# ortk95/planetmapper

Measured on NVIDIA B200. Metric: full-backplane Mpix/s (FP64) + mapped-cube voxels/s at 1-8 B200 vs host CPU, higher is better.
Workload: dtype f64

## Files before the change

### planetmapper_b200/csrc/backplane_kernels.cu

```cuda
#include "pm_device.cuh"
#include "pm_kernels.h"

#include <cstdlib>

namespace pm {

constexpr int kPerThread = 4;
#ifndef PM_IMG_PARAM_CTAS
#define PM_IMG_PARAM_CTAS 4
#endif
constexpr int kImgParamCtas = PM_IMG_PARAM_CTAS;

__device__ __forceinline__ int slot(uint64_t mask, int k) { return __popcll(mask & (bit(k) - 1ull)); }

struct PlaneOffsets {
    int64_t byte_off[PM_N_PLANES];
    int64_t frame_stride;
};
static PlaneOffsets make_plane_offsets(uint64_t mask, int64_t plane_stride) {
    PlaneOffsets po;
    int slot = 0;
    for (int k = 0; k < PM_N_PLANES; k++) {
        po.byte_off[k] = (int64_t)slot * plane_stride * (int64_t)sizeof(double);
        if (mask & bit(k)) slot++;
// ... 44 lines not shown
    const uint32_t j = (k + 1u) >> 1;
    if (j <= min(lo, hi)) return (k & 1u) ? centre + j : centre - j;
    return lo < hi ? k : n_tiles - 1u - k;
}
template <bool kSky, uint64_t kFixedMask>
__global__ void __launch_bounds__(kBlock, kImgParamCtas) backplanes_img_param_kernel(
    const __grid_constant__ FrameD fs, uint32_t nx, uint32_t npx, int per_thread, uint32_t centre_tile, uint64_t mask,
    const __grid_constant__ PlaneOffsets po, double *__restrict__ out) {
    img_tile<kSky, kFixedMask>(fs, centre_out_tile(blockIdx.x, gridDim.x, centre_tile), nx, npx, per_thread, mask,
                               po, out);
}

template <bool kSky, bool kRingAll>
__global__ void __launch_bounds__(kBlock, 4) backplanes_points_param_kernel(const __grid_constant__ FrameD fs,
                                                                            const double *__restrict__ x_in,
                                                                            const double *__restrict__ y_in,
                                                                            int64_t n, uint64_t mask,
                                                                            const __grid_constant__ PlaneOffsets po,
                                                                            double *__restrict__ out) {
    const int64_t first = (int64_t)blockIdx.x * (kBlock * kPerThread) + threadIdx.x;
#pragma unroll 1
    for (int r = 0; r < kPerThread; r++) {
        const int64_t idx = first + r * kBlock;
        if (idx >= n) break;
        PlaneSink sink{reinterpret_cast<char *>(out + idx), po};
        image_point<kSky, kRingAll>(fs, __ldg(x_in + idx), __ldg(y_in + idx), mask, sink);
    }
}

constexpr uint64_t kXYMapMask = bit(PM_PIXEL_X) | bit(PM_PIXEL_Y);

template <uint64_t kFixedMask>
__device__ __forceinline__ void map_tile(const FrameD &fs, const double *__restrict__ lon_in,
                                         const double *__restrict__ lat_in, int64_t n, uint64_t mask,
                                         const PlaneOffsets &po, double *__restrict__ out) {
    const int64_t first = (int64_t)blockIdx.x * (kBlock * kPerThread) + threadIdx.x;
#pragma unroll 1
    for (int r = 0; r < kPerThread; r++) {
        const int64_t idx = first + r * kBlock;
        if (idx >= n) break;
        PlaneSink sink{reinterpret_cast<char *>(out + idx), po};
        map_cell<kFixedMask>(fs, __ldg(lon_in + idx), __ldg(lat_in + idx), mask, sink);
    }
}

template <uint64_t kFixedMask>
__global__ void __launch_bounds__(kBlock, 4) backplanes_map_kernel(const PMFrame *__restrict__ frame,
                                                                   const double *__restrict__ lon_in,
                                                                   const double *__restrict__ lat_in,
                                                                   int64_t n, uint64_t mask,
                                                                   const __grid_constant__ PlaneOffsets po,
                                                                   double *__restrict__ out) {
    __shared__ FrameD fs;
    load_frame(fs, frame + blockIdx.y);
    map_tile<kFixedMask>(fs, lon_in, lat_in, n, mask, po, out + (int64_t)blockIdx.y * po.frame_stride);
}

template <uint64_t kFixedMask>
__global__ void __launch_bounds__(kBlock, 4) backplanes_map_param_kernel(const __grid_constant__ FrameD fs,
                                                                         const double *__restrict__ lon_in,
                                                                         const double *__restrict__ lat_in,
                                                                         int64_t n, uint64_t mask,
                                                                         const __grid_constant__ PlaneOffsets po,
                                                                         double *__restrict__ out) {
    map_tile<kFixedMask>(fs, lon_in, lat_in, n, mask, po, out);
}

__global__ void __launch_bounds__(kBlock, 4) xy2lonlat_kernel(const PMFrame *__restrict__ frame,
                                                              const double *__restrict__ xs,
                                                              const double *__restrict__ ys, int64_t n,
                                                              double *__restrict__ lon_out,
                                                              double *__restrict__ lat_out,
                                                              unsigned long long *__restrict__ n_missed) {
    __shared__ FrameD fs;
    load_frame(fs, frame);
    unsigned long long missed = 0;
    const int64_t first = (int64_t)blockIdx.x * (kBlock * kPerThread) + threadIdx.x;
#pragma unroll 1
    for (int r = 0; r < kPerThread; r++) {
        const int64_t idx = first + r * kBlock;
        if (idx >= n) break;
        const double x = xs[idx], y = ys[idx];
        double lon = NAN, lat = NAN;
        if (fabs(x) < INFINITY && fabs(y) < INFINITY) {
            if (!xy2lonlat_point(fs, x, y, lon, lat)) missed++;
        }
        lon_out[idx] = lon;
        lat_out[idx] = lat;
    }
    if (n_missed) {
        for (int o = 16; o > 0; o >>= 1) missed += __shfl_down_sync(0xffffffffu, missed, o);
        if ((threadIdx.x & 31) == 0 && missed) atomicAdd(n_missed, missed);
    }
}

__global__ void __launch_bounds__(kBlock, 4) lonlat2xy_kernel(const PMFrame *__restrict__ frame,
                                                              const double *__restrict__ lons,
                                                              const double *__restrict__ lats, int64_t n,
                                                              double alt, uint32_t flags,
                                                              double *__restrict__ x_out,
                                                              double *__restrict__ y_out) {
    __shared__ FrameD fs;
    load_frame(fs, frame);
    const int64_t first = (int64_t)blockIdx.x * (kBlock * kPerThread) + threadIdx.x;
#pragma unroll 1
    for (int r = 0; r < kPerThread; r++) {
        const int64_t idx = first + r * kBlock;
        if (idx >= n) break;
        const double lon = lons[idx], lat = lats[idx];
        double x = NAN, y = NAN;
        if (fabs(lon) < INFINITY && fabs(lat) < INFINITY)
            lonlat2xy_point(fs, lon, lat, alt, (flags & PM_FLAG_NOT_VISIBLE_NAN) != 0,
                            (flags & PM_FLAG_PLANETOCENTRIC) != 0, x, y);
        x_out[idx] = x;
        y_out[idx] = y;
    }
}

__global__ void __launch_bounds__(kBlock, 4) transform_kernel(const PMFrame *__restrict__ frame,
                                                              const __grid_constant__ TransformAux aux, int use_aux,
                                                              int src, int dst, const double *__restrict__ a_in,
                                                              const double *__restrict__ b_in, int64_t n, double alt,
                                                              uint32_t flags, double *__restrict__ a_out,
                                                              double *__restrict__ b_out,
                                                              unsigned long long *__restrict__ n_missed) {
    __shared__ FrameD fs;
    __shared__ TransformAux ax;
    load_frame(fs, frame);
    if (threadIdx.x < 13) {
        double v;
        if (use_aux) {
            v = threadIdx.x < 9 ? aux.Mc[threadIdx.x] : aux.km2ang[threadIdx.x - 9];
        } else if (threadIdx.x < 9) {
            v = fs.f.M[threadIdx.x];
        } else {
            const double *m = fs.f.ang2km;
            const double det = fma(m[0], m[3], -m[1] * m[2]);
            const int k = threadIdx.x - 9;
            v = (k == 0 ? m[3] : k == 1 ? -m[1] : k == 2 ? -m[2] : m[0]) / det;
        }
        (threadIdx.x < 9 ? ax.Mc[threadIdx.x] : ax.km2ang[threadIdx.x - 9]) = v;
    }
    __syncthreads();
    unsigned long long missed = 0;
    const int64_t first = (int64_t)blockIdx.x * (kBlock * kPerThread) + threadIdx.x;
#pragma unroll 1
    for (int r = 0; r < kPerThread; r++) {
        const int64_t idx = first + r * kBlock;
        if (idx >= n) break;
        double oa, ob;
        if (!point_transform(fs, ax, src, dst, a_in[idx], b_in[idx], alt, flags, oa, ob)) missed++;
        a_out[idx] = oa;
        b_out[idx] = ob;
    }
    if (n_missed) {
        for (int o = 16; o > 0; o >>= 1) missed += __shfl_down_sync(0xffffffffu, missed, o);
        if ((threadIdx.x & 31) == 0 && missed) atomicAdd(n_missed, missed);
    }
}

template <int kKind>
__global__ void __launch_bounds__(256) fp64_probe_kernel(double *out, const double *in, int iters, double m, double c) {
    double a[8], b[8], d[8];
#pragma unroll
    for (int i = 0; i < 8; i++) {
        a[i] = threadIdx.x * 1e-9 + i;
        b[i] = kKind ? in[(threadIdx.x + 2 * i + 1) & 63] : m;
        d[i] = kKind ? in[(threadIdx.x + 3 * i + 2) & 63] * 1e-12 : c;
    }
#pragma unroll 1
    for (int it = 0; it < iters; it++) {
#pragma unroll
        for (int i = 0; i < 8; i++) a[i] = kKind ? fma(a[i], b[i], d[i]) : fma(a[i], m, c);
    }
    double s = a[0] + a[1] + a[2] + a[3] + a[4] + a[5] + a[6] + a[7];
    if (s == 123.456) out[0] = s;
}

__global__ void math_probe_kernel(int kind, const double *__restrict__ a, const double *__restrict__ b,
                                  int64_t n, double *__restrict__ out) {
    const int64_t i = (int64_t)blockIdx.x * blockDim.x + threadIdx.x;
// ... 174 lines not shown
```

### planetmapper_b200/csrc/pm_device.cuh

```cuda
#pragma once

#include "../../include/pm_b200.h"
#include "pm_math.cuh"

namespace pm {

struct V3 {
    double x, y, z;
};

PM_HD V3 mk(double x, double y, double z) { return V3{x, y, z}; }
PM_HD V3 operator+(V3 a, V3 b) { return mk(a.x + b.x, a.y + b.y, a.z + b.z); }
PM_HD V3 operator-(V3 a, V3 b) { return mk(a.x - b.x, a.y - b.y, a.z - b.z); }
PM_HD V3 operator-(V3 a) { return mk(-a.x, -a.y, -a.z); }
PM_HD V3 operator*(double s, V3 a) { return mk(s * a.x, s * a.y, s * a.z); }
PM_HD double dot(V3 a, V3 b) { return fma(a.x, b.x, fma(a.y, b.y, a.z * b.z)); }
PM_HD V3 cross(V3 a, V3 b) {
    return mk(fma(a.y, b.z, -a.z * b.y), fma(a.z, b.x, -a.x * b.z), fma(a.x, b.y, -a.y * b.x));
}
PM_HD V3 mul3(V3 a, const double *s) { return mk(a.x * s[0], a.y * s[1], a.z * s[2]); }
PM_HD V3 axpy(double s, V3 b, V3 a) { return mk(fma(s, b.x, a.x), fma(s, b.y, a.y), fma(s, b.z, a.z)); }
PM_HD double norm(V3 a) { return fast_sqrt_lite(dot(a, a)); }
PM_HD V3 ld3(const double *p) { return mk(p[0], p[1], p[2]); }
PM_HD bool finite3(V3 a) { return fabs(a.x) < INFINITY && fabs(a.y) < INFINITY && fabs(a.z) < INFINITY; }
PM_HD V3 mxv(const double *m, V3 v) {
    return mk(fma(m[0], v.x, fma(m[1], v.y, m[2] * v.z)), fma(m[3], v.x, fma(m[4], v.y, m[5] * v.z)),
              fma(m[6], v.x, fma(m[7], v.y, m[8] * v.z)));
}
PM_HD V3 mtxv(const double *m, V3 v) {
    return mk(fma(m[0], v.x, fma(m[3], v.y, m[6] * v.z)), fma(m[1], v.x, fma(m[4], v.y, m[7] * v.z)),
              fma(m[2], v.x, fma(m[5], v.y, m[8] * v.z)));
}
PM_HD_NOINLINE double pymod360_slow(double a) {
    double r = ::fmod(a, 360.0);
    if (r != 0.0 && r < 0.0) r += 360.0;
    return r;
}
PM_HD double pymod360(double a) { return (a >= 0.0 && a < 360.0) ? a : pymod360_slow(a); }

struct FrameD {
    PMFrame f;
    double inv_c;
    double inv_r[3];
    double nw[3];
    double k[3];
    double wn;
    double rp;
    double e2, ep2;
    double inv_omf2;
    double omf;
    double P0b[3], VTb[3], ATb[3], VOb[3], S0b[3], VSb[3];
    double G[9];
    double y0[3];
    double y0m2;
    double As[6];
    double inv_kmpa;
    int biaxial;
    int pad_;
};

constexpr int kDeriveItems = 13;

PM_HD double ex_mul(double a, double b) {
#ifdef __CUDA_ARCH__
    return __dmul_rn(a, b);
#else
    return a * b;
#endif
}
PM_HD double ex_add(double a, double b) {
#ifdef __CUDA_ARCH__
    return __dadd_rn(a, b);
#else
    return a + b;
#endif
}
PM_HD double ex_div(double a, double b) {
#ifdef __CUDA_ARCH__
    return __ddiv_rn(a, b);
#else
    return a / b;
#endif
}
PM_HD double ex_sqrt(double a) {
#ifdef __CUDA_ARCH__
    return __dsqrt_rn(a);
#else
    return ::sqrt(a);
#endif
}
PM_HD double ex_dot3(double a0, double b0, double a1, double b1, double a2, double b2) {
    return ex_add(ex_add(ex_mul(a0, b0), ex_mul(a1, b1)), ex_mul(a2, b2));
}

PM_HD void derive_frame_item(FrameD &s, int item) {
    const PMFrame &f = s.f;
    if (item >= 3 && item <= 8) {
        const double *src = item == 3 ? f.P0 : item == 4 ? f.VT : item == 5 ? f.AT : item == 6 ? f.VO : item == 7 ? f.S0 : f.VS;
        double *dst = item == 3 ? s.P0b : item == 4 ? s.VTb : item == 5 ? s.ATb : item == 6 ? s.VOb : item == 7 ? s.S0b : s.VSb;
        for (int r = 0; r < 3; r++)
            dst[r] = ex_dot3(f.R0[3 * r], src[0], f.R0[3 * r + 1], src[1], f.R0[3 * r + 2], src[2]);
        if (item == 3) {
            for (int r = 0; r < 3; r++) s.y0[r] = ex_mul(-dst[r], ex_div(1.0, f.radii[r]));
            s.y0m2 = fma(s.y0[0], s.y0[0], fma(s.y0[1], s.y0[1], ex_mul(s.y0[2], s.y0[2])));
        }
    } else if (item >= 9 && item <= 11) {
        const int r = item - 9;
        for (int c = 0; c < 3; c++)
            s.G[3 * r + c] = ex_dot3(f.R0[3 * r], f.M[3 * c], f.R0[3 * r + 1], f.M[3 * c + 1], f.R0[3 * r + 2], f.M[3 * c + 2]);
    } else if (item == 12) {
        const double sc = kRpd / 3600.0;
        for (int c = 0; c < 3; c++) {
            s.As[c] = -ex_mul(f.A[c], sc);
            s.As[3 + c] = ex_mul(f.A[3 + c], sc);
        }
        s.inv_kmpa = ex_div(1.0, f.km_per_arcsec);
    } else if (item == 0) {
        s.inv_c = ex_div(1.0, f.clight);
        const double w2 = ex_dot3(f.omega[0], f.omega[0], f.omega[1], f.omega[1], f.omega[2], f.omega[2]);
        const double wn = ex_sqrt(w2);
        s.wn = wn;
        s.k[0] = wn > 0.0 ? ex_div(f.omega[0], wn) : 0.0;
        s.k[1] = wn > 0.0 ? ex_div(f.omega[1], wn) : 0.0;
        s.k[2] = wn > 0.0 ? ex_div(f.omega[2], wn) : 0.0;
    } else if (item == 1) {
        const double a = f.radii[0], b = f.radii[1], c = f.radii[2];
        s.inv_r[0] = ex_div(1.0, a);
        s.inv_r[1] = ex_div(1.0, b);
        s.inv_r[2] = ex_div(1.0, c);
        const double m = fmin(a, fmin(b, c));
        const double ma = ex_div(m, a), mb = ex_div(m, b), mc = ex_div(m, c);
        s.nw[0] = ex_mul(ma, ma);
        s.nw[1] = ex_mul(mb, mb);
        s.nw[2] = ex_mul(mc, mc);
    } else if (item == 2) {
        const double rp = ex_add(f.re, -ex_mul(f.f, f.re));
        const double re2 = ex_mul(f.re, f.re), rp2 = ex_mul(rp, rp);
        const double omf = ex_add(1.0, -f.f);
        s.rp = rp;
        s.e2 = ex_add(1.0, -ex_div(rp2, re2));
        s.ep2 = ex_add(ex_div(re2, rp2), -1.0);
        s.omf = omf;
        s.inv_omf2 = ex_div(1.0, ex_mul(omf, omf));
        s.biaxial = (f.radii[0] == f.radii[1]) && (f.re == f.radii[0]) && (fabs(rp - f.radii[2]) <= 4e-16 * f.radii[2]);
        s.pad_ = 0;
    }
}

#ifdef __CUDACC__
__device__ __forceinline__ void load_frame(FrameD &s, const PMFrame *__restrict__ g) {
    const double *src = reinterpret_cast<const double *>(g);
    double *dst = reinterpret_cast<double *>(&s.f);
    for (int i = threadIdx.x; i < PM_FRAME_NDOUBLES; i += blockDim.x) dst[i] = __ldg(src + i);
    __syncthreads();
    const int w = threadIdx.x >> 5, l = threadIdx.x & 31;
    int item = -1;
    if (blockDim.x >= 128) {
        if (w == 0 && l < 6) item = 3 + l;
        else if (w == 1 && l < 4) item = 9 + l;
        else if (w == 2 && l < 2) item = l;
        else if (w == 3 && l == 0) item = 2;
    } else if (threadIdx.x < kDeriveItems) {
        item = threadIdx.x;
    }
    if (item >= 0) derive_frame_item(s, item);
    __syncthreads();
}
#endif
inline void load_frame_host(FrameD &s, const PMFrame *g) {
    s.f = *g;
    for (int i = 0; i < kDeriveItems; i++) derive_frame_item(s, i);
}

#ifndef PM_GRAZING_COS2
#define PM_GRAZING_COS2 3.0e-3
#endif
constexpr double kGrazingCos2 = PM_GRAZING_COS2;

enum PixC {
    kPixDt1Min = 0,
    kPixGrazing = 1,
    kPixInv60 = 2,
    kPixInv3600 = 3,
    kPixRpd = 4,
    kPixBetaMax = 5,
};
PM_DEV_TABLE(kPixC, 6, 1.0e-6, kGrazingCos2, 1.0 / 60.0, 1.0 / 3600.0, kRpd, 1.0e-3)

struct Rot {
    double s, omc;
};
PM_HD Rot make_rot(const FrameD &fs, double dt) {
    const double th = fs.wn * dt;
    Rot r;
    if (fabs(th) < 0.001953125) {
        const double z = th * th;
        r.s = th * fma(z, fma(z, PM_T(kTinyC)[0], PM_T(kTinyC)[2]), 1.0);
        r.omc = z * fma(z, fma(z, -PM_T(kTinyC)[1], -PM_T(kTinyC)[3]), 0.5);
    } else {
        double sh, ch;
        sincos_lib(0.5 * th, &sh, &ch);
        r.s = 2.0 * sh * ch;
        r.omc = 2.0 * sh * sh;
    }
    return r;
}
PM_HD V3 spin_fwd(const FrameD &fs, Rot r, V3 w) {
    const V3 k = ld3(fs.k);
    const V3 c = cross(w, k);
    const double kw = dot(k, w);
    const V3 t = mk(fma(k.x, kw, -w.x), fma(k.y, kw, -w.y), fma(k.z, kw, -w.z));
    return axpy(r.omc, t, axpy(r.s, c, w));
}
PM_HD V3 spin_bwd_c(const FrameD &fs, Rot r, V3 u, V3 kxu) {
    const V3 k = ld3(fs.k);
    const double ku = dot(k, u);
    const V3 t = mk(fma(k.x, ku, -u.x), fma(k.y, ku, -u.y), fma(k.z, ku, -u.z));
    return axpy(r.omc, t, axpy(r.s, kxu, u));
}
PM_HD V3 spin_bwd(const FrameD &fs, Rot r, V3 u) { return spin_bwd_c(fs, r, u, cross(ld3(fs.k), u)); }
PM_HD V3 to_body(const FrameD &fs, Rot r, V3 v) { return spin_fwd(fs, r, mxv(fs.f.R0, v)); }
PM_HD V3 from_body(const FrameD &fs, Rot r, V3 u) { return mtxv(fs.f.R0, spin_bwd(fs, r, u)); }
PM_HD V3 target_pos_b(const FrameD &fs, double dt) {
    const double h = 0.5 * dt * dt;
    return mk(fma(fs.ATb[0], h, fma(fs.VTb[0], dt, fs.P0b[0])), fma(fs.ATb[1], h, fma(fs.VTb[1], dt, fs.P0b[1])),
              fma(fs.ATb[2], h, fma(fs.VTb[2], dt, fs.P0b[2])));
}

PM_HD void recrad_angles(V3 v, double &ra, double &dec) {
    dec = fast_atan2_xpos(v.z, fast_sqrt(fma(v.x, v.x, v.y * v.y)));
    double lon = fast_atan2(v.y, v.x);
    if (lon < 0.0) lon += kTwoPi;
    ra = lon;
}
PM_HD V3 radrec1(double ra, double dec) {
    double sr, cr, sd, cd;
    sincos_full(ra, sr, cr);
    sincos_full(dec, sd, cd);
    return mk(cr * cd, sr * cd, sd);
}
PM_HD double vsep(V3 a, V3 b) { return fast_atan2_ypos(norm(cross(a, b)), dot(a, b)); }

struct RayHit {
    V3 pp;
    double ixx;
    double a;
    double t;
    double cos2;
};
PM_HD bool surfpt_y(const FrameD &fs, V3 y, double ym2, V3 u, V3 &p, RayHit &hit) {
    const V3 x = mul3(u, fs.inv_r);
    const double xx = dot(x, x), yx = dot(y, x);
    if (!(xx > 0.0)) return false;
    const double ixx = fast_rcp(xx);
    const double a = -(yx * ixx);
    const V3 pp = axpy(a, x, y);
    const double pm2 = dot(pp, pp);
    if (!(pm2 < INFINITY)) return false;
    hit.pp = pp;
    hit.ixx = ixx;
    hit.a = a;
    hit.cos2 = 1.0 - pm2;
    double h;
    if (ym2 > 1.0) {
        if (pm2 > 1.0) return false;
        if (yx > 0.0) return false;
        h = -fast_sqrt_lite((1.0 - pm2) * ixx);
    } else if (ym2 == 1.0) {
        h = -a;
    } else {
        h = fast_sqrt_lite(fmax(0.0, 1.0 - pm2) * ixx);
    }
    hit.t = a + h;
    p = mul3(axpy(h, x, pp), fs.f.radii);
    return true;
}
PM_HD bool surfpt(const FrameD &fs, V3 o, V3 u, V3 &p, RayHit &hit) {
    const V3 y = mul3(o, fs.inv_r);
    return surfpt_y(fs, y, dot(y, y), u, p, hit);
}

struct Intercept {
    V3 p;
    V3 u;
    Rot r;
    double dt;
    double L;
    double lt;
};

PM_HD_NOINLINE bool sincpt_converge(const FrameD &fs, V3 u0, double &dt, V3 &p, double &range) {
    const PMFrame &f = fs.f;
    for (int it = 0; it < 8; it++) {
        const Rot r = make_rot(fs, dt);
        const V3 o = spin_fwd(fs, r, -target_pos_b(fs, dt));
        RayHit hit;
        if (!surfpt(fs, o, spin_fwd(fs, r, u0), p, hit)) return false;
        range = hit.t;
        const double t = dt + f.t_ref;
        const double t_new = f.et - hit.t * fs.inv_c;
        if (!(fabs(t_new - t) > 1.0e-17 * fabs(t_new))) break;
        dt = t_new - f.t_ref;
    }
    return true;
}

PM_HD bool sincpt(const FrameD &fs, V3 u0, Intercept &it) {
    const PMFrame &f = fs.f;
    V3 p1, p2;
    RayHit h1, h2;
    if (!surfpt_y(fs, ld3(fs.y0), fs.y0m2, u0, p1, h1)) return false;
    const double lt1 = h1.t * fs.inv_c;

    const double dt1 = (f.et - lt1) - f.t_ref;
    const Rot r1 = make_rot(fs, dt1);
    if (!surfpt(fs, spin_fwd(fs, r1, -target_pos_b(fs, dt1)), spin_fwd(fs, r1, u0), p2, h2)) return false;
    const double lt2 = h2.t * fs.inv_c;

    double dt = (f.et - lt2) - f.t_ref;
    V3 p;
    double L;
    if (fabs(dt1) > PM_T(kPixC)[kPixDt1Min] && h2.cos2 > PM_T(kPixC)[kPixGrazing]) {
        const double lam = fast_div_lite(dt - dt1, dt1 - (dt - dt1));
        dt = fma(lam, dt1, dt1) + f.t_ref;
        dt -= f.t_ref;
        const V3 pps = axpy(lam, h2.pp - h1.pp, h2.pp);
        const double hs = fast_sqrt_lite(fmax(1.0 - dot(pps, pps), 0.0) * fma(lam, h2.ixx - h1.ixx, h2.ixx));
        L = fma(lam, h2.a - h1.a, h2.a) - hs;
        it.r = make_rot(fs, dt);
        it.u = spin_fwd(fs, it.r, u0);
        p = axpy(-hs, it.u, mul3(pps, fs.f.radii));
    } else {
        double dt_c = dt, L_c;
        V3 p_c;
        if (!sincpt_converge(fs, u0, dt_c, p_c, L_c)) return false;
        dt = dt_c;
        p = p_c;
        L = L_c;
        it.r = make_rot(fs, dt);
        it.u = spin_fwd(fs, it.r, u0);
    }
    it.p = p;
    it.dt = dt;
    it.L = L;
    it.lt = L * fs.inv_c;
    return true;
}

PM_HD void geodetic_general(const FrameD &fs, double rho, double z, double &lat, double &alt) {
    const PMFrame &f = fs.f;
    if (f.f == 0.0) {
        lat = fast_atan2_xpos(z, rho);
        alt = fast_sqrt(fma(rho, rho, z * z)) - f.re;
        return;
    }
    double sb = f.re * z, cb = fs.rp * rho;
    double n = fast_rsqrt(fma(sb, sb, cb * cb) + sqrt_guard());
    sb *= n;
    cb *= n;
    double num = z, den = rho;
#pragma unroll 1
    for (int i = 0; i < 8; i++) {
        num = fma(fs.ep2 * fs.rp, sb * sb * sb, z);
        den = fma(-fs.e2 * f.re, cb * cb * cb, rho);
        double nsb = fs.omf * num, ncb = den;
        n = fast_rsqrt(fma(nsb, nsb, ncb * ncb) + sqrt_guard());
        nsb *= n;
        ncb *= n;
        const double change = fabs(nsb - sb) + fabs(ncb - cb);
// ... 63 lines not shown
PM_HD double local_solar_time(const PMFrame &f, double lon_deg) {
    double ang = f.lon_sign * (lon_deg * PM_T(kPixC)[kPixRpd]) - f.sun_lon_lst;
    if (f.prograde == 0.0) ang = -ang;
    const double k = floor(ang * PM_T(kMisc)[8]);
    ang = fma(-k, PM_T(kMisc)[7], ang);
    if (ang < 0.0) ang += PM_T(kMisc)[7];
    if (ang >= PM_T(kMisc)[7]) ang -= PM_T(kMisc)[7];
    double sec = fma(ang, 86400.0 / kTwoPi, 43200.0);
    if (sec >= 86400.0) sec -= 86400.0;
    const int isec = (int)sec;
    const int hr = isec / 3600, rem = isec - hr * 3600;
    const int mn = rem / 60, sc = rem - mn * 60;
    const double dm = (double)mn, ds = (double)sc;
    double qm = dm * PM_T(kPixC)[kPixInv60];
    qm = fma(fma(-60.0, qm, dm), PM_T(kPixC)[kPixInv60], qm);
    double qs = ds * PM_T(kPixC)[kPixInv3600];
    qs = fma(fma(-3600.0, qs, ds), PM_T(kPixC)[kPixInv3600], qs);
    return ((double)hr + qm) + qs;
}

PM_HD_NOINLINE double doppler_factor_closed(double beta) { return fast_sqrt(fast_div(1.0 + beta, 1.0 - beta)); }
PM_HD_NOINLINE double light_time_rate_closed(double a, double b, double c) { return fast_div(a - b, c + a); }
PM_HD double doppler_factor(const FrameD &fs, double rv) {
    const double beta = rv * fs.inv_c;
    if (fabs(beta) < PM_T(kPixC)[kPixBetaMax])
        return fma(beta, fma(beta, fma(beta, fma(beta, fma(beta, 0.375, 0.375), 0.5), 0.5), 1.0), 1.0);
    return doppler_factor_closed(beta);
}

PM_HD double radial_velocity(const FrameD &fs, double a, double b) {
    const double ac = a * fs.inv_c;
    double dlt = (a - b) * fs.inv_c * fma(ac, ac - 1.0, 1.0);
    if (!(fabs(ac) < PM_T(kPixC)[kPixBetaMax])) dlt = light_time_rate_closed(a, b, fs.f.clight);
    return fma(-dlt, a, a) - b;
}

struct Illum {
    double phase, incdnc, emissn, azimuth;
};
PM_HD void illum_angles(V3 n, V3 s, V3 e, bool want_az, Illum &out) {
    const V3 cse = cross(s, e), cns = cross(n, s), cne = cross(n, e);
    const double dse = dot(s, e), dns = dot(n, s), dne = dot(n, e);
    const double mns = norm(cns), mne = norm(cne);
    out.phase = fast_atan2_ypos(norm(cse), dse);
    out.incdnc = fast_atan2_ypos(mns, dns);
    out.emissn = fast_atan2_ypos(mne, dne);
    if (want_az) {
        const double nn = dot(n, n);
        const double a = fma(dse, nn, -dne * dns);
        out.azimuth = fast_atan2_ypos(fast_sqrt_pos(nn) * fabs(dot(n, cse)), -a);
    }
}

PM_HD void illum_at(const FrameD &fs, V3 p, V3 p0 , V3 e, Rot r, double dt, bool want_az,
                    Illum &out) {
    const PMFrame &f = fs.f;
    const double h = 0.5 * dt * dt;
    const V3 base = mk(fs.S0b[0] - fma(fs.ATb[0], h, fma(fs.VTb[0], dt, p0.x)),
                       fs.S0b[1] - fma(fs.ATb[1], h, fma(fs.VTb[1], dt, p0.y)),
                       fs.S0b[2] - fma(fs.ATb[2], h, fma(fs.VTb[2], dt, p0.z)));
    const V3 VSb = ld3(fs.VSb);
    V3 sv = axpy(dt, VSb, base);
    const double lts = fast_sqrt_pos(dot(sv, sv)) * fs.inv_c;
    sv = axpy(dt - (lts - f.lts0), VSb, base);
    const V3 s_b = spin_fwd(fs, r, sv);
    const V3 n = mul3(p, fs.nw);
    illum_angles(n, s_b, e, want_az, out);
}

struct PointGeom {
    V3 p0;
    V3 X0;
    Rot r;
    double dt, L, lt;
};
PM_HD void point_geom(const FrameD &fs, V3 p, PointGeom &g) {
    const PMFrame &f = fs.f;
    double lt = norm(ld3(fs.P0b) + p) * fs.inv_c;
#pragma unroll 1
    for (int pass = 0; pass < 2; pass++) {
        const double dt = (f.et - lt) - f.t_ref;
        const Rot r = make_rot(fs, dt);
        const V3 p0 = spin_bwd(fs, r, p);
        const V3 X0 = target_pos_b(fs, dt) + p0;
        const double L = norm(X0);
        lt = L * fs.inv_c;
        g.p0 = p0;
        g.X0 = X0;
        g.r = r;
        g.dt = dt;
        g.L = L;
        g.lt = lt;
    }
}
PM_HD double point_rv(const FrameD &fs, V3 p, const PointGeom &g) {
    const double iL = fast_rcp(g.L);
    const V3 ph0 = iL * g.X0;
    const V3 vt = axpy(g.dt, ld3(fs.ATb), ld3(fs.VTb));
    const V3 vrot0 = spin_bwd(fs, g.r, cross(ld3(fs.f.omega), p));
    const double a = dot(vt + vrot0, ph0);
    const double b = dot(ld3(fs.VOb), ph0);
    return radial_velocity(fs, a, b);
}

PM_HD V3 xy2ray_local(const FrameD &fs, double x, double y) {
    const double ra = fma(fs.As[0], x, fma(fs.As[1], y, fs.As[2]));
    const double dec = fma(fs.As[3], x, fma(fs.As[4], y, fs.As[5]));
    double sr, cr, sd, cd;
    sincos_small2(ra, dec, sr, cr, sd, cd);
    return mk(cr * cd, sr * cd, sd);
}

PM_HD void obsvec2angular(const PMFrame &f, V3 ov, double &ax, double &ay) {
    double ra, dec;
    recrad_angles(mxv(f.M, ov), ra, dec);
    double x = pymod360(-(ra * kDpr));
    if (x > 180.0) x -= 360.0;
    ax = x * 3600.0;
    ay = (dec * kDpr) * 3600.0;
}

PM_HD V3 targvec2obsvec(const FrameD &fs, V3 tv) {
    const PMFrame &f = fs.f;
    const V3 off = tv - ld3(f.sub_t);
    const double dist_offset = norm(ld3(f.sub_ray) + off) - f.sub_dist;
    const double sub_et = f.t_ref + f.sub_dt;
    const double tt = sub_et - dist_offset * fs.inv_c;
    const Rot r = make_rot(fs, tt - f.t_ref);
    return ld3(f.sub_obs) + from_body(fs, r, off);
}

PM_HD V3 obsvec2targvec(const FrameD &fs, V3 ov) {
    const PMFrame &f = fs.f;
    const V3 off = ov - ld3(f.sub_obs);
    const double dist_offset = norm(off - ld3(f.sub_ray)) - f.sub_dist;
    const double sub_et = f.t_ref + f.sub_dt;
    const double tt = sub_et - dist_offset * fs.inv_c;
    const Rot r = make_rot(fs, tt - f.t_ref);
    return ld3(f.sub_t) + to_body(fs, r, off);
}
// ... 58 lines not shown
    const bool try_disc = (mask & kSurfMask) && !(f.optimize_speed != 0.0 && fma(dx, dx, dy * dy) > f.r_cut2);
    V3 v = mk(nan, nan, nan);
    if (try_disc || (kSky && (mask & kSkyMask))) v = xy2ray_local(fs, x, y);
    V3 d2 = mk(nan, nan, nan);
    if (kSky && (mask & kSkyMask)) {
        const V3 d = mtxv(f.M, v);
        double ra, dec;
        recrad_angles(d, ra, dec);
        const double ra_deg = ra * kDpr, dec_deg = dec * kDpr;
        if (mask & bit(PM_RA)) out.put(PM_RA, ra_deg);
        if (mask & bit(PM_DEC)) out.put(PM_DEC, dec_deg);
        if (mask & (kKmMask | kLimbMask | kRingMask)) d2 = radrec1(ra_deg * kRpd, dec_deg * kRpd);
        if (mask & kKmMask) {
            double ax, ay;
            obsvec2angular(f, d2, ax, ay);
            const double kx = fma(f.ang2km[0], ax, f.ang2km[1] * ay);
            const double ky = fma(f.ang2km[2], ax, f.ang2km[3] * ay);
            if (mask & bit(PM_KM_X)) out.put(PM_KM_X, kx);
            if (mask & bit(PM_KM_Y)) out.put(PM_KM_Y, ky);
            if (mask & bit(PM_ANGULAR_X)) out.put(PM_ANGULAR_X, fast_div(kx, f.km_per_arcsec));
            if (mask & bit(PM_ANGULAR_Y)) out.put(PM_ANGULAR_Y, fast_div(ky, f.km_per_arcsec));
        }
    }

    bool on_disc = false;
    Intercept it;
    const V3 u0 = mxv(fs.G, v);
    if (try_disc) on_disc = sincpt(fs, u0, it);

    double v_dist = nan;
    if (on_disc) {
        const V3 p = it.p;
        if (mask & (kLonLatMask | kCentricMask)) {
            const double rho = fast_sqrt_lite(fma(p.x, p.x, p.y * p.y));
            const double lon_e = fast_atan2(p.y, p.x);
            if (mask & kLonLatMask) {
                double l = f.lon_sign * lon_e;
                if (l < 0.0) l += kTwoPi;
                const double v_lon = l * kDpr;
                double lat, alt;
                if (fs.biaxial) {
                    lat = fast_atan2_xpos(p.z * fs.inv_omf2, rho);
                } else {
                    geodetic_general(fs, rho, p.z, lat, alt);
                }
                if (mask & bit(PM_LON_GRAPHIC)) out.put(PM_LON_GRAPHIC, v_lon);
                if (mask & bit(PM_LAT_GRAPHIC)) out.put(PM_LAT_GRAPHIC, lat * kDpr);
                if (mask & bit(PM_LOCAL_SOLAR_TIME)) out.put(PM_LOCAL_SOLAR_TIME, local_solar_time(f, v_lon));
            }
            if (mask & bit(PM_LON_CENTRIC)) out.put(PM_LON_CENTRIC, lon_e * kDpr);
            if (mask & bit(PM_LAT_CENTRIC)) out.put(PM_LAT_CENTRIC, fast_atan2_xpos(p.z, rho) * kDpr);
        }
        if (mask & (kIllumMask | kStateMask | kRingMask)) {
            const V3 kxp = cross(ld3(fs.k), p);
            const V3 p0 = spin_bwd_c(fs, it.r, p, kxp);
            if (mask & kIllumMask) {
                Illum il;
                illum_at(fs, p, p0, -it.u, it.r, it.dt, (mask & bit(PM_AZIMUTH)) != 0, il);
                if (mask & bit(PM_PHASE)) out.put(PM_PHASE, il.phase * kDpr);
                if (mask & bit(PM_INCIDENCE)) out.put(PM_INCIDENCE, il.incdnc * kDpr);
                if (mask & bit(PM_EMISSION)) out.put(PM_EMISSION, il.emissn * kDpr);
                if (mask & bit(PM_AZIMUTH)) out.put(PM_AZIMUTH, il.azimuth * kDpr);
            }
            v_dist = it.lt * f.clight;
            if (mask & bit(PM_DISTANCE)) out.put(PM_DISTANCE, v_dist);
            if (mask & (bit(PM_RADIAL_VELOCITY) | bit(PM_DOPPLER))) {
                const V3 vt = axpy(it.dt, ld3(fs.ATb), ld3(fs.VTb));
                const double a = fma(fs.wn, dot(kxp, it.u), dot(vt, u0));
                const double b = dot(ld3(fs.VOb), u0);
                const double rv = radial_velocity(fs, a, b);
                if (mask & bit(PM_RADIAL_VELOCITY)) out.put(PM_RADIAL_VELOCITY, rv);
                if (mask & bit(PM_DOPPLER)) out.put(PM_DOPPLER, doppler_factor(fs, rv));
            }
        }
    } else {
        const uint64_t m = mask & (kLonLatMask | kCentricMask | kIllumMask | kStateMask);
#pragma unroll
        for (int k = 0; k <= PM_DOPPLER; k++)
            if ((kLonLatMask | kCentricMask | kIllumMask | kStateMask) & bit(k))
                if (m & bit(k)) out.put(k, nan);
    }

    if (kSky && (mask & kLimbMask)) {
        double llon, llat, ldist;
        limb_coordinates(fs, d2, llon, llat, ldist);
        if (mask & bit(PM_LIMB_DISTANCE)) out.put(PM_LIMB_DISTANCE, ldist);
        if (mask & bit(PM_LIMB_LON_GRAPHIC)) out.put(PM_LIMB_LON_GRAPHIC, llon);
        if (mask & bit(PM_LIMB_LAT_GRAPHIC)) out.put(PM_LIMB_LAT_GRAPHIC, llat);
    }
    if (kSky && (mask & kRingMask)) {
        double rad, rl, rd;
        ring_coordinates(fs, d2, rad, rl, rd);
        if (!kRingAll && rd > v_dist) rad = rl = rd = nan;
        if (mask & bit(PM_RING_RADIUS)) out.put(PM_RING_RADIUS, rad);
        if (mask & bit(PM_RING_LON_GRAPHIC)) out.put(PM_RING_LON_GRAPHIC, rl);
        if (mask & bit(PM_RING_DISTANCE)) out.put(PM_RING_DISTANCE, rd);
    }
}

template <bool kSky, bool kRingAll, class Sink>
PM_HD void image_point(const FrameD &fs, double x, double y, uint64_t mask_in, Sink &out) {
    if (fabs(x) < INFINITY && fabs(y) < INFINITY) {
        image_pixel<kSky, 0, kRingAll>(fs, x, y, mask_in, out);
        return;
    }
#pragma unroll 1
    for (int k = 0; k < PM_N_PLANES; k++)
        if (mask_in & bit(k)) out.put(k, k == PM_PIXEL_X ? x : (k == PM_PIXEL_Y ? y : (double)NAN));
}

template <uint64_t kFixedMask = 0, class Sink>
PM_HD void map_cell(const FrameD &fs, double lon_deg, double lat_deg, uint64_t mask_in, Sink &out) {
    const uint64_t mask = kFixedMask ? kFixedMask : mask_in;
    const PMFrame &f = fs.f;
    const double nan = NAN;
    const double lonm = (fabs(lon_deg) < INFINITY) ? pymod360(lon_deg) : nan;
    const double latm = (fabs(lat_deg) < INFINITY) ? lat_deg : nan;
    if (mask & bit(PM_LON_GRAPHIC)) out.put(PM_LON_GRAPHIC, lonm);
    if (mask & bit(PM_LAT_GRAPHIC)) out.put(PM_LAT_GRAPHIC, latm);
    const bool lon_ok = lonm == lonm;
    const bool ok = lon_ok && (latm == latm);
    if (mask & bit(PM_LOCAL_SOLAR_TIME))
        out.put(PM_LOCAL_SOLAR_TIME, lon_ok ? local_solar_time(f, lonm) : nan);

    double v_clon = nan, v_clat = nan, v_g = nan, v_i = nan, v_e = nan, v_az = nan, v_dist = nan, v_rv = nan,
           v_dop = nan, v_ra = nan, v_dec = nan, v_x = nan, v_y = nan, v_kx = nan, v_ky = nan, v_ax = nan,
           v_ay = nan;
    double limb_lon = nan, limb_lat = nan, limb_dist = nan, ring_rad = nan, ring_lon = nan, ring_dist = nan;
    if (ok) {
        const V3 tv = pgrrec0(fs, lonm * kRpd, latm * kRpd);
        if (mask & kCentricMask) {
            double lo, la;
            reclat_angles(tv, lo, la);
            v_clon = lo * kDpr;
            v_clat = la * kDpr;
        }
        PointGeom g;
        point_geom(fs, tv, g);
        Illum il;
        illum_at(fs, tv, g.p0, spin_fwd(fs, g.r, -g.X0), g.r, g.dt, (mask & bit(PM_AZIMUTH)) != 0, il);
        v_g = il.phase * kDpr;
        v_i = il.incdnc * kDpr;
        v_e = il.emissn * kDpr;
        if (mask & bit(PM_AZIMUTH)) v_az = il.azimuth * kDpr;
        v_dist = g.lt * f.clight;
        if (mask & (bit(PM_RADIAL_VELOCITY) | bit(PM_DOPPLER))) {
            v_rv = point_rv(fs, tv, g);
            v_dop = doppler_factor(fs, v_rv);
        }
        const bool visibl = il.emissn < kHalfPi, lit = il.incdnc < kHalfPi;
        const uint64_t vis_mask = bit(PM_RA) | bit(PM_DEC) | bit(PM_PIXEL_X) | bit(PM_PIXEL_Y) | kKmMask;
        const bool want_vis = visibl && (mask & vis_mask), want_lit = lit && (mask & (kLimbMask | kRingMask));
        if (want_vis || want_lit) {
            const V3 ov = targvec2obsvec(fs, tv);
            if (want_vis) {
                double ra, dec;
                recrad_angles(ov, ra, dec);
                v_ra = ra * kDpr;
                v_dec = dec * kDpr;
                if (mask & (vis_mask & ~(bit(PM_RA) | bit(PM_DEC)))) {
                    const V3 d2 = radrec1(v_ra * kRpd, v_dec * kRpd);
                    double ax, ay;
                    obsvec2angular(f, d2, ax, ay);
                    const double x = fma(f.Ainv[0], ax, fma(f.Ainv[1], ay, f.Ainv[2]));
                    const double y = fma(f.Ainv[3], ax, fma(f.Ainv[4], ay, f.Ainv[5]));
                    if ((-0.5 < x && x < f.nx - 0.5) && (-0.5 < y && y < f.ny - 0.5)) {
                        v_x = x;
                        v_y = y;
                    }
                    v_kx = fma(f.ang2km[0], ax, f.ang2km[1] * ay);
                    v_ky = fma(f.ang2km[2], ax, f.ang2km[3] * ay);
                    if (mask & (bit(PM_ANGULAR_X) | bit(PM_ANGULAR_Y))) {
                        v_ax = fast_div(v_kx, f.km_per_arcsec);
                        v_ay = fast_div(v_ky, f.km_per_arcsec);
                    }
                }
            }
            if (lit && (mask & kLimbMask)) limb_coordinates(fs, ov, limb_lon, limb_lat, limb_dist);
            if (lit && (mask & kRingMask)) {
                ring_coordinates(fs, ov, ring_rad, ring_lon, ring_dist);
                if (ring_dist > v_dist) ring_rad = ring_lon = ring_dist = nan;
            }
        }
    }
    if (mask & bit(PM_LON_CENTRIC)) out.put(PM_LON_CENTRIC, v_clon);
    if (mask & bit(PM_LAT_CENTRIC)) out.put(PM_LAT_CENTRIC, v_clat);
    if (mask & bit(PM_RA)) out.put(PM_RA, v_ra);
    if (mask & bit(PM_DEC)) out.put(PM_DEC, v_dec);
    if (mask & bit(PM_PIXEL_X)) out.put(PM_PIXEL_X, v_x);
    if (mask & bit(PM_PIXEL_Y)) out.put(PM_PIXEL_Y, v_y);
    if (mask & bit(PM_KM_X)) out.put(PM_KM_X, v_kx);
    if (mask & bit(PM_KM_Y)) out.put(PM_KM_Y, v_ky);
    if (mask & bit(PM_ANGULAR_X)) out.put(PM_ANGULAR_X, v_ax);
// ... 189 lines not shown
```

Before: 29930.

## Replace per-pixel observer and sun light-time geometry with precomputed epoch cubic polynomials

Result: faster. 31630 (median of 6 runs) (+5.7%).

```diff
diff --git a/planetmapper_b200/csrc/backplane_kernels.cu b/planetmapper_b200/csrc/backplane_kernels.cu
--- a/planetmapper_b200/csrc/backplane_kernels.cu
+++ b/planetmapper_b200/csrc/backplane_kernels.cu
@@ -120,7 +120,7 @@
                                                                    const __grid_constant__ PlaneOffsets po,
                                                                    double *__restrict__ out) {
     __shared__ FrameD fs;
-    load_frame(fs, frame + blockIdx.y);
+    load_frame(fs, frame + blockIdx.y, kFixedMask != kXYMapMask);
     map_tile<kFixedMask>(fs, lon_in, lat_in, n, mask, po, out + (int64_t)blockIdx.y * po.frame_stride);
 }
 
@@ -169,7 +169,7 @@
                                                               double *__restrict__ x_out,
                                                               double *__restrict__ y_out) {
     __shared__ FrameD fs;
-    load_frame(fs, frame);
+    load_frame(fs, frame, alt != 0.0 && (flags & PM_FLAG_NOT_VISIBLE_NAN));
     const int64_t first = (int64_t)blockIdx.x * (kBlock * kPerThread) + threadIdx.x;
 #pragma unroll 1
     for (int r = 0; r < kPerThread; r++) {
@@ -194,7 +194,8 @@
                                                               unsigned long long *__restrict__ n_missed) {
     __shared__ FrameD fs;
     __shared__ TransformAux ax;
-    load_frame(fs, frame);
+    load_frame(fs, frame, dst == PM_COORD_LONLAT || dst == PM_COORD_CENTRIC ||
+                              (src == PM_COORD_LONLAT && alt != 0.0 && (flags & PM_FLAG_NOT_VISIBLE_NAN)));
     if (threadIdx.x < 13) {
         double v;
         if (use_aux) {
diff --git a/planetmapper_b200/csrc/pm_device.cuh b/planetmapper_b200/csrc/pm_device.cuh
--- a/planetmapper_b200/csrc/pm_device.cuh
+++ b/planetmapper_b200/csrc/pm_device.cuh
@@ -55,11 +55,17 @@
     double y0m2;
     double As[6];
     double inv_kmpa;
+    double Yc[9];
+    double Sc[9];
+    double lts_e0, lts_e1;
+    double sun_u[3];
+    double dt_poly_max;
     int biaxial;
     int pad_;
 };
 
 constexpr int kDeriveItems = 13;
+constexpr int kEpochItems = 4;
 
 PM_HD double ex_mul(double a, double b) {
 #ifdef __CUDA_ARCH__
@@ -91,6 +97,67 @@
 }
 PM_HD double ex_dot3(double a0, double b0, double a1, double b1, double a2, double b2) {
     return ex_add(ex_add(ex_mul(a0, b0), ex_mul(a1, b1)), ex_mul(a2, b2));
+}
+PM_HD double ex_dot(V3 a, V3 b) { return ex_dot3(a.x, b.x, a.y, b.y, a.z, b.z); }
+PM_HD double ex_norm(V3 a) { return ex_sqrt(ex_dot(a, a)); }
+PM_HD V3 ex_sub(V3 a, V3 b) { return mk(ex_add(a.x, -b.x), ex_add(a.y, -b.y), ex_add(a.z, -b.z)); }
+PM_HD V3 ex_axpy(double s, V3 b, V3 a) {
+    return mk(ex_add(a.x, ex_mul(s, b.x)), ex_add(a.y, ex_mul(s, b.y)), ex_add(a.z, ex_mul(s, b.z)));
+}
+
+PM_HD void ex_spin_cubic(V3 k, double wn, V3 w0, V3 w1, V3 w2, V3 c[3]) {
+    const auto C = [&](V3 w) {
+        return mk(ex_add(ex_mul(w.y, k.z), -ex_mul(w.z, k.y)), ex_add(ex_mul(w.z, k.x), -ex_mul(w.x, k.z)),
+                  ex_add(ex_mul(w.x, k.y), -ex_mul(w.y, k.x)));
+    };
+    const auto D = [&](V3 w) {
+        const double kw = ex_dot(k, w);
+        return mk(ex_add(ex_mul(k.x, kw), -w.x), ex_add(ex_mul(k.y, kw), -w.y), ex_add(ex_mul(k.z, kw), -w.z));
+    };
+    const double h2 = ex_mul(0.5, ex_mul(wn, wn)), h3 = ex_mul(ex_mul(wn, ex_mul(wn, wn)), 1.0 / 6.0);
+    const V3 C0 = C(w0), C1 = C(w1), C2 = C(w2);
+    c[0] = ex_axpy(wn, C0, w1);
+    c[1] = ex_axpy(h2, D(w0), ex_axpy(wn, C1, w2));
+    c[2] = ex_axpy(-h3, C0, ex_axpy(h2, D(w1), mk(ex_mul(wn, C2.x), ex_mul(wn, C2.y), ex_mul(wn, C2.z))));
+}
+PM_HD double ex_cubic_tail(double wn, double d, double W0, double W1, double W2) {
+    const double t = ex_mul(wn, d), t2 = ex_mul(t, t);
+    const double v1 = ex_mul(W1, d), v2 = ex_mul(W2, ex_mul(d, d));
+    const double s = ex_mul(ex_mul(t2, t2), ex_add(1.0 / 24.0, ex_mul(t, 1.0 / 120.0)));
+    return ex_add(ex_add(ex_mul(s, ex_add(ex_add(W0, v1), v2)), ex_mul(ex_mul(t2, ex_mul(t, 1.0 / 6.0)), ex_add(v1, v2))),
+                  ex_mul(ex_mul(t2, 0.5), v2));
+}
+
+
+constexpr double kPolyTol = 0.05 * 0x1p-53;
+constexpr double kSunDirTol = 1.0e-14;
+
+PM_HD double derive_dt_poly_max(const FrameD &s) {
+    const PMFrame &f = s.f;
+    const double wn = s.wn, inv_c = s.inv_c;
+    const V3 P0b = ld3(s.P0b), VTb = ld3(s.VTb), ATb = ld3(s.ATb), S0b = ld3(s.S0b), VSb = ld3(s.VSb);
+    const V3 DVb = ex_sub(VSb, VTb);
+    const double nP = ex_norm(P0b), nVT = ex_norm(VTb), nAT = ex_norm(ATb), nS = ex_norm(S0b), nVS = ex_norm(VSb),
+                 nDV = ex_norm(DVb);
+    const double rmin = fmin(f.radii[0], fmin(f.radii[1], f.radii[2]));
+    const double rmax = fmax(fmax(f.radii[0], fmax(f.radii[1], f.radii[2])), f.re);
+    const double inv_S = ex_div(1.0, nS);
+    const double tolY = ex_mul(ex_mul(kPolyTol, nP), ex_div(rmin, rmax)), tolS = ex_mul(kPolyTol, nS);
+    const double e0 = fabs(ex_add(ex_mul(nS, inv_c), -f.lts0)), e1 = fabs(ex_mul(ex_dot(S0b, DVb), ex_mul(inv_S, inv_c)));
+    const double vs = ex_mul(nVS, inv_S);
+    const auto sun_err = [&](double d) {
+        const double D = ex_add(ex_add(ex_mul(ex_mul(rmax, rmax), inv_S), ex_mul(ex_mul(rmax, ex_add(wn, ex_mul(nDV, inv_S))), d)),
+                                ex_mul(ex_add(ex_mul(ex_mul(nDV, nDV), inv_S), nAT), ex_mul(d, d)));
+        const double eps = ex_add(ex_add(e0, ex_mul(e1, d)), ex_mul(ex_add(rmax, D), inv_c));
+        return ex_mul(ex_add(ex_mul(D, inv_c), ex_mul(eps, ex_mul(wn, d))), vs);
+    };
+    if (!(ex_mul(4.0, rmax) <= nS) || !(sun_err(0.0) <= kSunDirTol)) return -1.0;
+    double d = ex_mul(1.25, ex_mul(rmax, inv_c));
+    for (int i = 0; i < 64; i++, d = ex_mul(0.5, d))
+        if (ex_mul(wn, d) <= 0x1p-10 && ex_cubic_tail(wn, d, nP, nVT, ex_mul(0.5, nAT)) <= tolY &&
+            ex_cubic_tail(wn, d, nS, nDV, ex_mul(0.5, nAT)) <= tolS && sun_err(d) <= kSunDirTol)
+            return d;
+    return -1.0;
 }
 
 PM_HD void derive_frame_item(FrameD &s, int item) {
@@ -123,6 +190,28 @@
         s.k[0] = wn > 0.0 ? ex_div(f.omega[0], wn) : 0.0;
         s.k[1] = wn > 0.0 ? ex_div(f.omega[1], wn) : 0.0;
         s.k[2] = wn > 0.0 ? ex_div(f.omega[2], wn) : 0.0;
+    } else if (item == 13 || item == 14) {
+        const bool y = item == 13;
+        const V3 VTb = ld3(s.VTb), w2 = mk(-0.5 * s.ATb[0], -0.5 * s.ATb[1], -0.5 * s.ATb[2]);
+        V3 c[3];
+        if (y) ex_spin_cubic(ld3(s.k), s.wn, -ld3(s.P0b), -VTb, w2, c);
+        else ex_spin_cubic(ld3(s.k), s.wn, ld3(s.S0b), ex_sub(ld3(s.VSb), VTb), w2, c);
+        double *dst = y ? s.Yc : s.Sc;
+        for (int j = 0; j < 3; j++) {
+            dst[3 * j] = y ? ex_mul(c[j].x, s.inv_r[0]) : c[j].x;
+            dst[3 * j + 1] = y ? ex_mul(c[j].y, s.inv_r[1]) : c[j].y;
+            dst[3 * j + 2] = y ? ex_mul(c[j].z, s.inv_r[2]) : c[j].z;
+        }
+    } else if (item == 15) {
+        const V3 S0b = ld3(s.S0b);
+        const double nS = ex_norm(S0b), q = ex_div(s.inv_c, nS);
+        s.lts_e0 = ex_add(ex_mul(nS, s.inv_c), -f.lts0);
+        s.lts_e1 = ex_mul(ex_dot(S0b, ex_sub(ld3(s.VSb), ld3(s.VTb))), q);
+        s.sun_u[0] = ex_mul(S0b.x, q);
+        s.sun_u[1] = ex_mul(S0b.y, q);
+        s.sun_u[2] = ex_mul(S0b.z, q);
+    } else if (item == 16) {
+        s.dt_poly_max = derive_dt_poly_max(s);
     } else if (item == 1) {
         const double a = f.radii[0], b = f.radii[1], c = f.radii[2];
         s.inv_r[0] = ex_div(1.0, a);
@@ -148,7 +237,7 @@
 }
 
 #ifdef __CUDACC__
-__device__ __forceinline__ void load_frame(FrameD &s, const PMFrame *__restrict__ g) {
+__device__ __forceinline__ void load_frame(FrameD &s, const PMFrame *__restrict__ g, bool epoch = true) {
     const double *src = reinterpret_cast<const double *>(g);
     double *dst = reinterpret_cast<double *>(&s.f);
     for (int i = threadIdx.x; i < PM_FRAME_NDOUBLES; i += blockDim.x) dst[i] = __ldg(src + i);
@@ -164,12 +253,17 @@
         item = threadIdx.x;
     }
     if (item >= 0) derive_frame_item(s, item);
+    if (!epoch && threadIdx.x == 0) s.dt_poly_max = -1.0;
+    __syncthreads();
+    if (!epoch) return;
+    item = blockDim.x >= 128 ? (l == 0 ? kDeriveItems + w : -1) : (int)threadIdx.x + kDeriveItems;
+    if (item >= kDeriveItems && item < kDeriveItems + kEpochItems) derive_frame_item(s, item);
     __syncthreads();
 }
 #endif
 inline void load_frame_host(FrameD &s, const PMFrame *g) {
     s.f = *g;
-    for (int i = 0; i < kDeriveItems; i++) derive_frame_item(s, i);
+    for (int i = 0; i < kDeriveItems + kEpochItems; i++) derive_frame_item(s, i);
 }
 
 #ifndef PM_GRAZING_COS2
@@ -190,19 +284,21 @@
 struct Rot {
     double s, omc;
 };
+PM_HD Rot rot_series(double th) {
+    const double z = th * th;
+    Rot r;
+    r.s = th * fma(z, fma(z, PM_T(kTinyC)[0], PM_T(kTinyC)[2]), 1.0);
+    r.omc = z * fma(z, fma(z, -PM_T(kTinyC)[1], -PM_T(kTinyC)[3]), 0.5);
+    return r;
+}
 PM_HD Rot make_rot(const FrameD &fs, double dt) {
     const double th = fs.wn * dt;
+    if (fabs(th) < 0.001953125) return rot_series(th);
+    double sh, ch;
+    sincos_lib(0.5 * th, &sh, &ch);
     Rot r;
-    if (fabs(th) < 0.001953125) {
-        const double z = th * th;
-        r.s = th * fma(z, fma(z, PM_T(kTinyC)[0], PM_T(kTinyC)[2]), 1.0);
-        r.omc = z * fma(z, fma(z, -PM_T(kTinyC)[1], -PM_T(kTinyC)[3]), 0.5);
-    } else {
-        double sh, ch;
-        sincos_lib(0.5 * th, &sh, &ch);
-        r.s = 2.0 * sh * ch;
-        r.omc = 2.0 * sh * sh;
-    }
+    r.s = 2.0 * sh * ch;
+    r.omc = 2.0 * sh * sh;
     return r;
 }
 PM_HD V3 spin_fwd(const FrameD &fs, Rot r, V3 w) {
@@ -212,19 +308,39 @@
     const V3 t = mk(fma(k.x, kw, -w.x), fma(k.y, kw, -w.y), fma(k.z, kw, -w.z));
     return axpy(r.omc, t, axpy(r.s, c, w));
 }
-PM_HD V3 spin_bwd_c(const FrameD &fs, Rot r, V3 u, V3 kxu) {
+PM_HD V3 spin_bwd(const FrameD &fs, Rot r, V3 u) {
     const V3 k = ld3(fs.k);
     const double ku = dot(k, u);
     const V3 t = mk(fma(k.x, ku, -u.x), fma(k.y, ku, -u.y), fma(k.z, ku, -u.z));
-    return axpy(r.omc, t, axpy(r.s, kxu, u));
-}
-PM_HD V3 spin_bwd(const FrameD &fs, Rot r, V3 u) { return spin_bwd_c(fs, r, u, cross(ld3(fs.k), u)); }
+    return axpy(r.omc, t, axpy(r.s, cross(k, u), u));
+}
 PM_HD V3 to_body(const FrameD &fs, Rot r, V3 v) { return spin_fwd(fs, r, mxv(fs.f.R0, v)); }
 PM_HD V3 from_body(const FrameD &fs, Rot r, V3 u) { return mtxv(fs.f.R0, spin_bwd(fs, r, u)); }
 PM_HD V3 target_pos_b(const FrameD &fs, double dt) {
     const double h = 0.5 * dt * dt;
     return mk(fma(fs.ATb[0], h, fma(fs.VTb[0], dt, fs.P0b[0])), fma(fs.ATb[1], h, fma(fs.VTb[1], dt, fs.P0b[1])),
               fma(fs.ATb[2], h, fma(fs.VTb[2], dt, fs.P0b[2])));
+}
+PM_HD V3 epoch_poly(V3 c0, const double *c, double dt) {
+    return mk(fma(dt, fma(dt, fma(dt, c[6], c[3]), c[0]), c0.x), fma(dt, fma(dt, fma(dt, c[7], c[4]), c[1]), c0.y),
+              fma(dt, fma(dt, fma(dt, c[8], c[5]), c[2]), c0.z));
+}
+struct ObserverAt {
+    V3 y;
+    Rot r;
+};
+PM_HD_NOINLINE ObserverAt observer_scaled_exact(const FrameD &fs, double dt) {
+    ObserverAt o;
+    o.r = make_rot(fs, dt);
+    o.y = mul3(spin_fwd(fs, o.r, -target_pos_b(fs, dt)), fs.inv_r);
+    return o;
+}
+PM_HD ObserverAt observer_scaled(const FrameD &fs, double dt) {
+    if (!(fabs(dt) <= fs.dt_poly_max)) return observer_scaled_exact(fs, dt);
+    ObserverAt o;
+    o.r = rot_series(fs.wn * dt);
+    o.y = epoch_poly(ld3(fs.y0), fs.Yc, dt);
+    return o;
 }
 
 PM_HD void recrad_angles(V3 v, double &ra, double &dec) {
@@ -313,8 +429,8 @@
     const double lt1 = h1.t * fs.inv_c;
 
     const double dt1 = (f.et - lt1) - f.t_ref;
-    const Rot r1 = make_rot(fs, dt1);
-    if (!surfpt(fs, spin_fwd(fs, r1, -target_pos_b(fs, dt1)), spin_fwd(fs, r1, u0), p2, h2)) return false;
+    const ObserverAt o1 = observer_scaled(fs, dt1);
+    if (!surfpt_y(fs, o1.y, dot(o1.y, o1.y), spin_fwd(fs, o1.r, u0), p2, h2)) return false;
     const double lt2 = h2.t * fs.inv_c;
 
     double dt = (f.et - lt2) - f.t_ref;
@@ -484,24 +600,29 @@
     }
 }
 
-PM_HD void illum_at(const FrameD &fs, V3 p, V3 p0 , V3 e, Rot r, double dt, bool want_az,
-                    Illum &out) {
-    const PMFrame &f = fs.f;
+PM_HD_NOINLINE V3 sun_from_point_exact(const FrameD &fs, V3 p, Rot r, double dt) {
+    const V3 VSb = ld3(fs.VSb);
+    const V3 p0 = spin_bwd(fs, r, p);
     const double h = 0.5 * dt * dt;
     const V3 base = mk(fs.S0b[0] - fma(fs.ATb[0], h, fma(fs.VTb[0], dt, p0.x)),
                        fs.S0b[1] - fma(fs.ATb[1], h, fma(fs.VTb[1], dt, p0.y)),
                        fs.S0b[2] - fma(fs.ATb[2], h, fma(fs.VTb[2], dt, p0.z)));
-    const V3 VSb = ld3(fs.VSb);
     V3 sv = axpy(dt, VSb, base);
     const double lts = fast_sqrt_pos(dot(sv, sv)) * fs.inv_c;
-    sv = axpy(dt - (lts - f.lts0), VSb, base);
-    const V3 s_b = spin_fwd(fs, r, sv);
+    sv = axpy(dt - (lts - fs.f.lts0), VSb, base);
+    return spin_fwd(fs, r, sv);
+}
+PM_HD V3 sun_from_point(const FrameD &fs, V3 p, Rot r, double dt) {
+    if (!(fabs(dt) <= fs.dt_poly_max)) return sun_from_point_exact(fs, p, r, dt);
+    const double eps = fma(dt, fs.lts_e1, fs.lts_e0) - dot(ld3(fs.sun_u), p);
+    return axpy(-eps, ld3(fs.VSb), epoch_poly(ld3(fs.S0b), fs.Sc, dt) - p);
+}
+PM_HD void illum_at(const FrameD &fs, V3 p, V3 e, Rot r, double dt, bool want_az, Illum &out) {
     const V3 n = mul3(p, fs.nw);
-    illum_angles(n, s_b, e, want_az, out);
+    illum_angles(n, sun_from_point(fs, p, r, dt), e, want_az, out);
 }
 
 struct PointGeom {
-    V3 p0;
     V3 X0;
     Rot r;
     double dt, L, lt;
@@ -517,7 +638,6 @@
         const V3 X0 = target_pos_b(fs, dt) + p0;
         const double L = norm(X0);
         lt = L * fs.inv_c;
-        g.p0 = p0;
         g.X0 = X0;
         g.r = r;
         g.dt = dt;
@@ -682,11 +802,9 @@
             if (mask & bit(PM_LAT_CENTRIC)) out.put(PM_LAT_CENTRIC, fast_atan2_xpos(p.z, rho) * kDpr);
         }
         if (mask & (kIllumMask | kStateMask | kRingMask)) {
-            const V3 kxp = cross(ld3(fs.k), p);
-            const V3 p0 = spin_bwd_c(fs, it.r, p, kxp);
             if (mask & kIllumMask) {
                 Illum il;
-                illum_at(fs, p, p0, -it.u, it.r, it.dt, (mask & bit(PM_AZIMUTH)) != 0, il);
+                illum_at(fs, p, -it.u, it.r, it.dt, (mask & bit(PM_AZIMUTH)) != 0, il);
                 if (mask & bit(PM_PHASE)) out.put(PM_PHASE, il.phase * kDpr);
                 if (mask & bit(PM_INCIDENCE)) out.put(PM_INCIDENCE, il.incdnc * kDpr);
                 if (mask & bit(PM_EMISSION)) out.put(PM_EMISSION, il.emissn * kDpr);
@@ -696,7 +814,7 @@
             if (mask & bit(PM_DISTANCE)) out.put(PM_DISTANCE, v_dist);
             if (mask & (bit(PM_RADIAL_VELOCITY) | bit(PM_DOPPLER))) {
                 const V3 vt = axpy(it.dt, ld3(fs.ATb), ld3(fs.VTb));
-                const double a = fma(fs.wn, dot(kxp, it.u), dot(vt, u0));
+                const double a = fma(fs.wn, dot(cross(ld3(fs.k), p), it.u), dot(vt, u0));
                 const double b = dot(ld3(fs.VOb), u0);
                 const double rv = radial_velocity(fs, a, b);
                 if (mask & bit(PM_RADIAL_VELOCITY)) out.put(PM_RADIAL_VELOCITY, rv);
@@ -768,7 +886,7 @@
         PointGeom g;
         point_geom(fs, tv, g);
         Illum il;
-        illum_at(fs, tv, g.p0, spin_fwd(fs, g.r, -g.X0), g.r, g.dt, (mask & bit(PM_AZIMUTH)) != 0, il);
+        illum_at(fs, tv, spin_fwd(fs, g.r, -g.X0), g.r, g.dt, (mask & bit(PM_AZIMUTH)) != 0, il);
         v_g = il.phase * kDpr;
         v_i = il.incdnc * kDpr;
         v_e = il.emissn * kDpr;
```
